# sp-uhh/audio-visual-vad

Hardware: AMD Instinct MI355X
Metric: AV frame-pairs/sec (fwd+bwd) (higher is better)
Workload: dtype f32; 1 GPU; AV_net fused training step (WaveNet-W0 encoder + ResNet-18 trunk + concat + 2xLSTM1024 + FC, masked BCE, backward, RCCL all-reduce, fused Adam): BASELINE configs[3]/[4] per-GPU shard; per_gpu_frame_pairs=1024, global_frame_pairs=1024, sequences_per_gpu=64, parallelism=dp1, reserved_cus=0, reported_block=median

## Files before the change

audio-visual-vad_amd/csrc/wavenet.hip:

```cpp
#include "gemm_api.h"
#include "wn_block.h"
#include "wn_tail.h"

namespace {

static inline int grid1(long n) { long b = (n + 255) / 256; return (int)(b > 8192 ? 8192 : (b < 1 ? 1 : b)); }

__global__ void conv1d_fwd_generic(const float* __restrict__ x, const float* __restrict__ w, const float* __restrict__ bias,
                                   const float* __restrict__ res, float* __restrict__ y, int B, int Cin, int Cout, int Lin,
                                   int Lout, int fw, int dil, int relu_in, int res_off, int res_L) {
  const long n = (long)B * Cout * Lout;
  for (long i = (long)blockIdx.x * blockDim.x + threadIdx.x; i < n; i += (long)gridDim.x * blockDim.x) {
    const int t = (int)(i % Lout);
    const int co = (int)((i / Lout) % Cout);
    const int b = (int)(i / ((long)Lout * Cout));
    float acc = bias ? bias[co] : 0.f;
    const float* xb = x + (long)b * Cin * Lin + t;
    const float* wr = w + (long)co * Cin * fw;
    for (int ci = 0; ci < Cin; ++ci)
      for (int k = 0; k < fw; ++k) {
        float v = xb[(long)ci * Lin + k * dil];
        if (relu_in) v = fmaxf(v, 0.f);
        acc = fmaf(wr[ci * fw + k], v, acc);
      }
// ... 29 lines not shown
  const int c = blockIdx.x;
  float s = 0.f;
  for (int b = blockIdx.y; b < B; b += gridDim.y) {
    const float* p = dy + ((long)b * C + c) * L;
    for (int t = threadIdx.x; t < L; t += 256) s += p[t];
  }
  sm[threadIdx.x] = s;
  __syncthreads();
  for (int o = 128; o > 0; o >>= 1) {
    if (threadIdx.x < o) sm[threadIdx.x] += sm[threadIdx.x + o];
    __syncthreads();
  }
  if (threadIdx.x == 0) db[c] += sm[0];
}

__global__ void __launch_bounds__(256)
    narrow_conv1d_grads(const float* __restrict__ dy, const float* __restrict__ x, float* __restrict__ part,
                        int B, int Cout, int Cin, int Lout, int Lin, int fw) {
  __shared__ float sm[5][256];
  const int co = blockIdx.x, nw = Cin * fw;
  float acc[5] = {0.f, 0.f, 0.f, 0.f, 0.f};
  for (int b = blockIdx.y; b < B; b += gridDim.y) {
    const float* p = dy + ((long)b * Cout + co) * Lout;
    const float* xb = x + (long)b * Cin * Lin;
    for (int t = threadIdx.x; t < Lout; t += 256) {
      const float g = p[t];
      acc[4] += g;
#pragma unroll
      for (int j = 0; j < 4; ++j)
        if (j < nw) acc[j] = fmaf(g, xb[(long)(j / fw) * Lin + t + (j % fw)], acc[j]);
    }
  }
#pragma unroll
  for (int j = 0; j < 5; ++j) sm[j][threadIdx.x] = acc[j];
  __syncthreads();
  for (int o = 128; o > 0; o >>= 1) {
    if (threadIdx.x < o)
#pragma unroll
      for (int j = 0; j < 5; ++j) sm[j][threadIdx.x] += sm[j][threadIdx.x + o];
    __syncthreads();
  }
  if (threadIdx.x < 5) part[((long)blockIdx.y * Cout + co) * 5 + threadIdx.x] = sm[threadIdx.x][0];
}
__global__ void narrow_conv1d_grads_sum(const float* __restrict__ part, int ny, int Cout, int nw, float* __restrict__ dw,
                                        float* __restrict__ db) {
  const int i = blockIdx.x * blockDim.x + threadIdx.x;
  if (i >= Cout * 5) return;
  const int co = i / 5, j = i - co * 5;
  float s = 0.f;
  for (int y = 0; y < ny; ++y) s += part[((long)y * Cout + co) * 5 + j];
  if (j < 4) { if (j < nw && dw) dw[(long)co * nw + j] += s; }
  else if (db) db[co] += s;
}

template <int MODE>
__global__ void __launch_bounds__(256)
    wn_block_fwd_mfma(const float* __restrict__ s_in, const float* __restrict__ w_dil, const float* __restrict__ b_dil,
                      const float* __restrict__ w_dense, const float* __restrict__ b_dense, float* __restrict__ s_out,
                      float* __restrict__ z_out, int B, int Lin, int dil) {
  static_assert(MODE == 0 || MODE == 2, "s_out only, or z only");
  const int lane = threadIdx.x & 63;
  const int li = lane & 31, lh = lane >> 5;
  const int Lo = Lin - dil;
  const int tiles_per_seq = tiles_per_sequence<32>(Lo);
  const long ntiles = (long)B * tiles_per_seq;
// ... 831 lines not shown
  if (threadIdx.x >= 32 || nslab <= 0) return;
  if (i < 2048) { if (tab.dW_dil[l]) tab.dW_dil[l][(i & 1023) * 2 + (i >> 10)] += s; }
  else if (i < 3072) { if (tab.dW_dense[l]) tab.dW_dense[l][i - 2048] += s; }
  else if (i < 3104) { if (tab.db_dil[l]) tab.db_dil[l][i - 3072] += s; }
  else if (tab.db_dense[l]) tab.db_dense[l][i - 3104] += s;
}

struct Plan {
  int n;
  int L[66];
  size_t s[66];
  size_t z, dz, ga, gb, dzt;
  size_t zs[66];
  size_t slab;
  size_t gslab;
  size_t total;
};
static int make_plan(const avvad_wavenet_desc* d, Plan* p) {
  if (!d || d->n_layers < 0 || d->n_layers > 64 || d->B <= 0 || d->fw < 1 || d->qc < 1 || d->R < 1 || d->D < 1 ||
      d->Bn < 1 || d->P < 1 || (d->n_layers > 0 && !d->dilations_h))
    return AVVAD_EINVAL;
  p->n = d->n_layers;
  p->L[0] = d->L - (d->fw - 1);
  for (int i = 0; i < p->n; ++i) p->L[i + 1] = p->L[i] - d->dilations_h[i] * (d->fw - 1);
  if (p->L[p->n] < 1) return AVVAD_EINVAL;
  size_t off = 0;
  auto take = [&](size_t n) { size_t o = off; off += align_up(n, 64); return o; };
  const size_t B = d->B;
  if (d->save_for_backward) {
    for (int i = 0; i <= p->n; ++i) p->s[i] = take(B * d->R * p->L[i]);
    const size_t big = B * (size_t)(d->R > d->D ? d->R : d->D) * p->L[0];
    p->z = take(big); p->dz = take(big); p->ga = take(big); p->gb = take(big);
    p->dzt = take(B * d->Bn * p->L[p->n]);
    {
      const size_t zb = (d->R == 32 && d->D == 32 && d->fw == 2 && p->n > 0) ? take(B * d->D * p->L[1]) : 0;
      for (int i = 0; i < p->n; ++i) p->zs[i] = zb;
    }
    {
      const bool perlayer = d->R == 32 && d->D == 32 && d->fw == 2;
      const size_t a = (size_t)WG_MAXBLK * WG_SLAB * (perlayer ? (size_t)p->n : 1), b2 = (size_t)TAIL_MAXBLK * tail_slab_floats(d->Bn);
      p->slab = take(a > b2 ? a : b2);
    }
    p->gslab = take(igemm::SLAB_FLOATS);
  } else {
    for (int i = 0; i < p->n; ++i) p->zs[i] = 0;
    const size_t a = take(B * d->R * p->L[0]), b2 = take(B * d->R * p->L[0]);
    for (int i = 0; i <= p->n; ++i) p->s[i] = (i & 1) ? b2 : a;
    p->z = take(B * d->D * p->L[0]);
    p->dz = p->ga = p->gb = p->dzt = 0;
  }
  p->total = off;
  return AVVAD_OK;
}

static inline bool mfma_shape(const avvad_wavenet_desc* d) { return d->R == 32 && d->D == 32 && d->fw == 2; }
static inline bool buf_ok(int B, int Lin) {
  return avvad_tune().wn_flat != 1 && (long)Lin * 32 * 4 + 4096 < (1L << 31) && (long)B * cdiv(Lin, 32) < (1L << 31);
}

enum class FwdForm { FLAT, BUF, OCC, WIDE, DMA };
enum class DxForm { FLAT, BUF, OCC };
enum class BwdForm { RESIDENT, OCC, TRANSPOSED, UNFUSED };
enum class TailFwdForm { GENERIC, MFMA1, MFMA4 };
enum class TailBwdForm { PAIR, FUSED, MFMA, GENERIC };
struct FwdChoice { FwdForm form; int grid; };
struct DxChoice { DxForm form; int grid; };
struct BwdChoice { BwdForm form; int grid; int grid_z, grid_dz; };
struct TailFwdChoice { TailFwdForm form; int grid; };
struct TailBwdChoice { TailBwdForm form; int grid; };
// ... 84 lines not shown
  const int ktiles = cdiv(K, igemm::BK);
  int split = 1024 / (cdiv(Cout, 64) * cdiv(Cin * fw, 64));
  if (split > ktiles) split = ktiles;
  if (split < 1) split = 1;
  igemm::RowSegK a{dy, Lout, (long)Cout * Lout, Cout, (int)K, Lout, 0, 0, 1, 0};
  igemm::RowSegK b{x, Lin, (long)Cin * Lin, Cin * fw, (int)K, Lout, 0, relu_in, fw, dil};
  igemm::EpiStore e{dw, (long)Cin * fw, nullptr, 1};
  return igemm::launch<64, 64>(a, b, e, Cout, Cin * fw, (int)K, split, s, slab);
}

static void bias_grad(const float* dy, float* db, int B, int C, int L, hipStream_t s) {
  if (!db) return;
  hipLaunchKernelGGL(chan_sum_acc, dim3(C, 1), dim3(256), 0, s, dy, db, B, C, L);
}

static void launch_tail_fwd(const float* sN, const float* wb, const float* bb, float* out, int B, int R, int Bn, int Lv, int P,
                            hipStream_t s) {
  const TailFwdChoice c = tail_fwd_form(B, R, Bn, P);
  switch (c.form) {
    case TailFwdForm::MFMA4: hipLaunchKernelGGL(tail_fwd_mfma<4>, dim3(c.grid), dim3(256), 0, s, sN, wb, bb, out, B, Bn, Lv, P); break;
    case TailFwdForm::MFMA1: hipLaunchKernelGGL(tail_fwd_mfma<1>, dim3(c.grid), dim3(256), 0, s, sN, wb, bb, out, B, Bn, Lv, P); break;
    case TailFwdForm::GENERIC: hipLaunchKernelGGL(tail_fwd_generic, dim3(P, B), dim3(256), 0, s, sN, wb, bb, out, R, Bn, Lv, P); break;
  }
}

static int launch_tail_bwd(const float* sN, const float* wb, const float* bb, const float* dout, float* dW, float* db, float* dS,
                           float* dzt, float* slab, float* gslab, int B, int R, int Bn, int Lv, int P, hipStream_t s) {
  const TailBwdChoice c = tail_bwd_form(B, Lv, R, Bn, P, dW || db);
  int rc;
  if (c.form == TailBwdForm::PAIR || c.form == TailBwdForm::FUSED) {
    const bool pair = c.form == TailBwdForm::PAIR;
    const size_t lds = (size_t)tail_fused_lds_floats(Bn, pair ? 2 : 1) * sizeof(float);
    if ((rc = pair ? allow_large_lds<tail_bwd_wgrad_pair<8>>(lds, lds) : allow_large_lds<tail_bwd_wgrad_mfma<8>>(lds, lds))) return rc;
    hipLaunchKernelGGL(pair ? tail_bwd_wgrad_pair<8> : tail_bwd_wgrad_mfma<8>, dim3(c.grid), dim3(pair ? 512 : 256), lds, s, sN, wb,
                       bb, dout, dS, slab, B, Lv, P);
    hipLaunchKernelGGL(tail_wgrad_reduce, dim3(cdiv(tail_slab_floats(Bn), 32)), dim3(256), 0, s, slab, c.grid, Bn, dW, db);
    return AVVAD_OK;
  }
  if (c.form == TailBwdForm::MFMA)
    hipLaunchKernelGGL(tail_bwd_mfma, dim3(c.grid), dim3(256), (size_t)tail_wimg_floats(Bn) * sizeof(float), s, sN, wb, bb, dout,
                       dzt, dS, B, Bn, Lv, P);
  else
    hipLaunchKernelGGL(tail_bwd_dz_generic, dim3(grid1((long)B * Bn * Lv)), dim3(256), 0, s, sN, wb, bb, dout, dzt, B, R, Bn, Lv, P);
  if (dW && (rc = wgrad_conv1d(dzt, sN, dW, B, Bn, R, Lv, Lv, 1, 1, 0, s, gslab))) return rc;
  bias_grad(dzt, db, B, Bn, Lv, s);
  if (c.form == TailBwdForm::GENERIC)
    hipLaunchKernelGGL(conv1d_bwd_data_generic, dim3(grid1((long)B * R * Lv)), dim3(256), 0, s, dzt, wb, (const float*)nullptr,
                       (const float*)nullptr, dS, B, R, Bn, Lv, Lv, 1, 1, 0, 0);
  return AVVAD_OK;
}

}

extern "C" size_t avvad_wavenet_workspace(const avvad_wavenet_desc* d) {
  Plan p;
  if (make_plan(d, &p)) return 0;
  return p.total * sizeof(float);
}

extern "C" int avvad_wavenet_fwd(const float* wave, const avvad_wavenet_params* prm, float* out, const avvad_wavenet_desc* d,
                                 void* wsv, size_t ws_bytes, avvad_stream_t sv) {
  AVVAD_ENTER();
  Plan p;
  if (!wave || !prm || !out || !wsv || ws_misaligned(wsv) || make_plan(d, &p)) return AVVAD_EINVAL;
  if (ws_bytes < p.total * sizeof(float)) return AVVAD_EWORKSPACE;
  hipStream_t s = (hipStream_t)sv;
  float* ws = (float*)wsv;
  const int B = d->B, R = d->R, D = d->D, fw = d->fw;
  hipLaunchKernelGGL(conv1d_fwd_generic, dim3(grid1((long)B * R * p.L[0])), dim3(256), 0, s, wave, prm->causal_w,
                     d->use_bias ? prm->causal_b : (const float*)nullptr, (const float*)nullptr, ws + p.s[0], B, d->qc, R,
                     d->L, p.L[0], fw, 1, 0, 0, 0);
  for (int i = 0; i < p.n; ++i) {
    const int dil = d->dilations_h[i];
    const float* bd = d->use_bias ? prm->dil_b_h[i] : nullptr;
    const float* be = d->use_bias ? prm->dense_b_h[i] : nullptr;
    if (mfma_shape(d)) {
      launch_block_fwd(ws + p.s[i], prm->dil_w_h[i], bd, prm->dense_w_h[i], be, ws + p.s[i + 1], B, p.L[i], dil, s);
    } else {
      float* z = ws + p.z;
      hipLaunchKernelGGL(conv1d_fwd_generic, dim3(grid1((long)B * D * p.L[i + 1])), dim3(256), 0, s, ws + p.s[i],
                         prm->dil_w_h[i], bd, (const float*)nullptr, z, B, R, D, p.L[i], p.L[i + 1], fw, dil, 1, 0, 0);
      hipLaunchKernelGGL(conv1d_fwd_generic, dim3(grid1((long)B * R * p.L[i + 1])), dim3(256), 0, s, z, prm->dense_w_h[i], be,
                         ws + p.s[i], ws + p.s[i + 1], B, D, R, p.L[i + 1], p.L[i + 1], 1, 1, 1, p.L[i] - p.L[i + 1], p.L[i]);
    }
  }
  launch_tail_fwd(ws + p.s[p.n], prm->bott_w, d->use_bias ? prm->bott_b : (const float*)nullptr, out, B, R, d->Bn, p.L[p.n],
                  d->P, s);
  AVVAD_LAUNCH_CHECK();
  return AVVAD_OK;
}

extern "C" int avvad_wavenet_block_fwd(const float* s_in, const float* w_dil, const float* b_dil, const float* w_dense,
                                       const float* b_dense, float* s_out, int B, int Lin, int dil, avvad_stream_t sv) {
  AVVAD_ENTER();
  if (!s_in || !w_dil || !w_dense || !s_out || B <= 0 || dil < 1 || Lin - dil < 1) return AVVAD_EINVAL;
  launch_block_fwd(s_in, w_dil, b_dil, w_dense, b_dense, s_out, B, Lin, dil, (hipStream_t)sv);
  AVVAD_LAUNCH_CHECK();
  return AVVAD_OK;
}

extern "C" int avvad_wavenet_bwd(const float* wave, const avvad_wavenet_params* prm, const float* dout,
                                 const avvad_wavenet_grads* g, float* dwave, const avvad_wavenet_desc* d, void* wsv,
                                 size_t ws_bytes, avvad_stream_t sv) {
  AVVAD_ENTER();
  Plan p;
  if (!wave || !prm || !dout || !g || !wsv || ws_misaligned(wsv) || make_plan(d, &p) || !d->save_for_backward) return AVVAD_EINVAL;
  if (ws_bytes < p.total * sizeof(float)) return AVVAD_EWORKSPACE;
  hipStream_t s = (hipStream_t)sv;
  float* ws = (float*)wsv;
  const int B = d->B, R = d->R, D = d->D, fw = d->fw, Bn = d->Bn;
  int rc;
  float* Z = ws + p.z;
  float* DZ = ws + p.dz;
  float* GA = ws + p.ga;
  float* GB = ws + p.gb;
  if ((rc = launch_tail_bwd(ws + p.s[p.n], prm->bott_w, d->use_bias ? prm->bott_b : (const float*)nullptr, dout, g->bott_w,
                            d->use_bias ? g->bott_b : (float*)nullptr, GA, ws + p.dzt, ws + p.slab, ws + p.gslab, B, R, Bn,
                            p.L[p.n], d->P, s)))
    return rc;
  WgradTab wtab;
  bool any_slab = false;
  for (int l = 0; l < WN_MAXL; ++l) {
    wtab.slab[l] = nullptr; wtab.nslab[l] = 0;
    wtab.dW_dil[l] = wtab.db_dil[l] = wtab.dW_dense[l] = wtab.db_dense[l] = nullptr;
  }
  auto note_slabs = [&](int i, float* slab_i, int wb) {
    wtab.slab[i] = slab_i; wtab.nslab[i] = wb;
    wtab.dW_dil[i] = g->dil_w_h[i]; wtab.dW_dense[i] = g->dense_w_h[i];
    wtab.db_dil[i] = d->use_bias ? g->dil_b_h[i] : (float*)nullptr;
    wtab.db_dense[i] = d->use_bias ? g->dense_b_h[i] : (float*)nullptr;
    any_slab = true;
// ... 47 lines not shown
          break;
      }
    } else {
      if (g->dense_w_h[i] && (rc = wgrad_conv1d(GA, Zi, g->dense_w_h[i], B, R, D, Lo, Lo, 1, 1, 1, s, ws + p.gslab))) return rc;
      if (d->use_bias) bias_grad(GA, g->dense_b_h[i], B, R, Lo, s);
      hipLaunchKernelGGL(conv1d_bwd_data_generic, dim3(grid1((long)B * D * Lo)), dim3(256), 0, s, GA, prm->dense_w_h[i], Zi,
                         (const float*)nullptr, DZ, B, D, R, Lo, Lo, 1, 1, 0, 0);
      if (g->dil_w_h[i] && (rc = wgrad_conv1d(DZ, si, g->dil_w_h[i], B, D, R, Lo, Li, fw, dil, 1, s, ws + p.gslab))) return rc;
      if (d->use_bias) bias_grad(DZ, g->dil_b_h[i], B, D, Lo, s);
      hipLaunchKernelGGL(conv1d_bwd_data_generic, dim3(grid1((long)B * R * Li)), dim3(256), 0, s, DZ, prm->dil_w_h[i], si, GA,
                         GB, B, R, D, Li, Lo, fw, dil, Li - Lo, Lo);
    }
    float* t = GA; GA = GB; GB = t;
  }
  if (any_slab) hipLaunchKernelGGL(wn_wgrad_reduce_all, dim3(WG_SLAB / 32, p.n), dim3(256), 0, s, wtab);
  if (d->qc * fw <= 4) {
    if (g->causal_w || (d->use_bias && g->causal_b))
    {
      const int ny = B < 32 ? B : 32;
      float* part = ws + p.gslab;
      hipLaunchKernelGGL(narrow_conv1d_grads, dim3(R, ny), dim3(256), 0, s, GA, wave, part, B, R, d->qc, p.L[0], d->L, fw);
      hipLaunchKernelGGL(narrow_conv1d_grads_sum, dim3(cdiv(R * 5, 256)), dim3(256), 0, s, part, ny, R, d->qc * fw, g->causal_w,
                         d->use_bias ? g->causal_b : (float*)nullptr);
    }
  } else {
    if (g->causal_w && (rc = wgrad_conv1d(GA, wave, g->causal_w, B, R, d->qc, p.L[0], d->L, fw, 1, 0, s, ws + p.gslab))) return rc;
    if (d->use_bias) bias_grad(GA, g->causal_b, B, R, p.L[0], s);
  }
  if (dwave)
    hipLaunchKernelGGL(conv1d_bwd_data_generic, dim3(grid1((long)B * d->qc * d->L)), dim3(256), 0, s, GA, prm->causal_w,
                       (const float*)nullptr, (const float*)nullptr, dwave, B, d->qc, R, d->L, p.L[0], fw, 1, 0, 0);
  AVVAD_LAUNCH_CHECK();
  return AVVAD_OK;
}
```

audio-visual-vad_amd/csrc/wn_tail.h:

```cpp
#pragma once
#include "common.h"

namespace {

constexpr int TAIL_MAXBLK = 256;
constexpr int TAIL_PITCH = 33;
constexpr int TAIL_TILE = 32 * TAIL_PITCH;
constexpr int tail_wimg_floats(int Bn) { return Bn * TAIL_PITCH; }
constexpr int tail_slab_floats(int Bn) { return Bn * 32 + Bn; }
constexpr int tail_fused_lds_floats(int Bn, int WPT) {
  return tail_wimg_floats(Bn) + tail_slab_floats(Bn) + 4 * WPT * 2 * TAIL_TILE + (WPT == 2 ? 4 * TAIL_TILE : 0);
}

__device__ __forceinline__ void pool_bin(int p, int Lv, int P, int& a, int& e) {
  a = (int)(((long)p * Lv) / P);
  e = (int)((((long)(p + 1)) * Lv + P - 1) / P);
}
__device__ __forceinline__ void stage_tail_weights(float* img, const float* __restrict__ wb, int Bn, int tid, int nthreads) {
  for (int i = tid; i < Bn * 32; i += nthreads) img[(i >> 5) * TAIL_PITCH + (i & 31)] = wb[i];
}
struct PoolWindow { int pb[3]; float pc[3]; };
__device__ __forceinline__ PoolWindow pool_window(int t, bool ok, int Lv, int P) {
  PoolWindow w;
  const int c0 = ok ? (int)(((long)t * P) / Lv) : 0;
#pragma unroll
  for (int j = 0; j < 3; ++j) {
    const int p = c0 - 1 + j;
    int a = 0, e = 0;
    const bool in = ok && p >= 0 && p < P;
    if (in) pool_bin(p, Lv, P, a, e);
    const bool hit = in && t >= a && t < e;
    w.pb[j] = hit ? p : 0;
    w.pc[j] = hit ? 1.f / (float)(e - a) : 0.f;
  }
  return w;
}
__device__ __forceinline__ f32x16 tail_z_tile(const float* wl, const float* __restrict__ bb, int nb, const float (&x)[16], int li, int lh) {
  f32x16 accZ;
#pragma unroll
  for (int r = 0; r < 16; ++r) accZ[r] = bb ? bb[nb + mfma32_row(r, lh)] : 0.f;
  float wz[16];
#pragma unroll
  for (int k = 0; k < 16; ++k) wz[k] = wl[(nb + li) * TAIL_PITCH + 2 * k + lh];
#pragma unroll
  for (int k = 0; k < 16; ++k) accZ = mfma32(wz[k], x[k], accZ);
  return accZ;
}
template <class Fetch>
__device__ __forceinline__ void tail_dz_tile(const f32x16& accZ, Fetch fetch, float (&dz)[16]) {
#pragma unroll
  for (int r = 0; r < 16; ++r) { const float g = fetch(r); dz[r] = accZ[r] > 0.f ? g : 0.f; }
}
__device__ __forceinline__ void tail_wt_frag(const float* wl, int nb, int li, int lh, float (&wt)[16]) {
#pragma unroll
  for (int k = 0; k < 16; ++k) wt[k] = wl[(nb + mfma32_row(k, lh)) * TAIL_PITCH + li];
}
__device__ __forceinline__ void tail_ds_product(f32x16& accS, const float (&wt)[16], const float (&dz)[16]) {
#pragma unroll
  for (int r = 0; r < 16; ++r) accS = mfma32(wt[r], dz[r], accS);
}
template <bool DLAYOUT>
__device__ __forceinline__ void tile_to_fragment(float* T, const float (&v)[16], float (&f)[16], int li, int lh) {
  __builtin_amdgcn_wave_barrier();
#pragma unroll
  for (int k = 0; k < 16; ++k) T[(DLAYOUT ? mfma32_row(k, lh) : 2 * k + lh) * TAIL_PITCH + li] = v[k];
  __builtin_amdgcn_wave_barrier();
// ... 53 lines not shown
    const float* sb = s + (long)b * R * Lv + t;
    for (int c = 0; c < R; ++c) z = fmaf(wb[(long)bn * R + c], sb[(long)c * Lv], z);
    float g = 0.f;
    if (z > 0.f) {
      const int p0 = (int)(((long)t * P) / Lv), p1 = (int)((((long)t + 1) * P + Lv - 1) / Lv);
      for (int p = p0; p < p1; ++p) {
        int a, e;
        pool_bin(p, Lv, P, a, e);
        g += dout[((long)b * Bn + bn) * P + p] / (float)(e - a);
      }
    }
    dz[i] = g;
  }
}

template <int NT>
__global__ void __launch_bounds__(256)
    tail_fwd_mfma(const float* __restrict__ s, const float* __restrict__ wb, const float* __restrict__ bb,
                  float* __restrict__ out, int B, int Bn, int Lv, int P) {
  const int lane = threadIdx.x & 63;
  const int li = lane & 31, lh = lane >> 5;
  const int ngrp = Bn / (32 * NT);
  const long nitems = (long)B * P * ngrp;
  const long nwaves = ((long)gridDim.x * blockDim.x) >> 6;
  for (long item = ((long)blockIdx.x * blockDim.x + threadIdx.x) >> 6; item < nitems; item += nwaves) {
    const int grp = (int)(item % ngrp);
    const int p = (int)((item / ngrp) % P);
    const int b = (int)(item / ((long)ngrp * P));
    const int bn0 = grp * 32 * NT;
    int a, e;
    pool_bin(p, Lv, P, a, e);
    float w[NT][16], bias[NT], sum[NT];
#pragma unroll
    for (int n = 0; n < NT; ++n) {
#pragma unroll
      for (int k = 0; k < 16; ++k) w[n][k] = wb[(long)(bn0 + n * 32 + li) * 32 + 2 * k + lh];
      bias[n] = bb ? bb[bn0 + n * 32 + li] : 0.f;
      sum[n] = 0.f;
    }
    const float* sp = s + (long)b * 32 * Lv;
    for (int t0 = a; t0 < e; t0 += 32) {
      const int t = t0 + li;
      const bool ok = t < e;
      const int tcl = ok ? t : a;
      float x[16];
#pragma unroll
      for (int k = 0; k < 16; ++k) x[k] = sp[(long)(2 * k + lh) * Lv + tcl];
#pragma unroll
      for (int k = 0; k < 16; ++k) x[k] = ok ? x[k] : 0.f;
#pragma unroll
      for (int n = 0; n < NT; ++n) {
        f32x16 acc = {};
#pragma unroll
        for (int k = 0; k < 16; ++k) acc = mfma32(x[k], w[n][k], acc);
#pragma unroll
        for (int r = 0; r < 16; ++r)
          if (t0 + mfma32_row(r, lh) < e) sum[n] += relu1(acc[r] + bias[n]);
      }
    }
    const float inv = 1.f / (float)(e - a);
#pragma unroll
    for (int n = 0; n < NT; ++n) {
      const float v = sum[n] + __shfl_xor(sum[n], 32, 64);
      if (lh == 0) out[((long)b * Bn + bn0 + n * 32 + li) * P + p] = v * inv;
    }
  }
}

__global__ void __launch_bounds__(256)
    tail_bwd_mfma(const float* __restrict__ s, const float* __restrict__ wb, const float* __restrict__ bb,
                  const float* __restrict__ dout, float* __restrict__ dzt, float* __restrict__ dS, int B, int Bn, int Lv, int P) {
  const int lane = threadIdx.x & 63;
  const int li = lane & 31, lh = lane >> 5;
  const int tiles_per_seq = (Lv + 31) >> 5;
  const long ntiles = (long)B * tiles_per_seq;
  const long nwaves = ((long)gridDim.x * blockDim.x) >> 6;
  extern __shared__ float wl[];
  stage_tail_weights(wl, wb, Bn, threadIdx.x, 256);
  __syncthreads();
  for (long tile = ((long)blockIdx.x * blockDim.x + threadIdx.x) >> 6; tile < ntiles; tile += nwaves) {
    const int b = (int)(tile / tiles_per_seq);
    const int t = (int)(tile - (long)b * tiles_per_seq) * 32 + li;
    const bool ok = t < Lv;
    const float* sp = s + (long)b * 32 * Lv + (ok ? t : 0);
    float x[16];
#pragma unroll
    for (int k = 0; k < 16; ++k) x[k] = sp[(long)(2 * k + lh) * Lv];
#pragma unroll
    for (int k = 0; k < 16; ++k) x[k] = ok ? x[k] : 0.f;
    const PoolWindow pw = pool_window(t, ok, Lv, P);
    f32x16 accS = {};
    for (int nb = 0; nb < Bn; nb += 32) {
      const f32x16 accZ = tail_z_tile(wl, bb, nb, x, li, lh);
      float dz[16];
      tail_dz_tile(accZ, [&](int r) {
        const long o = ((long)b * Bn + nb + mfma32_row(r, lh)) * P;
        float g = 0.f;
#pragma unroll
        for (int j = 0; j < 3; ++j) g = fmaf(dout[o + pw.pb[j]], pw.pc[j], g);
        return g;
      }, dz);
#pragma unroll
      for (int r = 0; r < 16; ++r)
        if (ok) dzt[((long)b * Bn + nb + mfma32_row(r, lh)) * Lv + t] = dz[r];
      float wt[16];
      tail_wt_frag(wl, nb, li, lh, wt);
      tail_ds_product(accS, wt, dz);
    }
#pragma unroll
    for (int r = 0; r < 16; ++r)
      if (ok) dS[((long)b * 32 + mfma32_row(r, lh)) * Lv + t] = accS[r];
  }
}

template <int NBT, int WPT>
__device__ __forceinline__ void tail_bwd_wgrad_body(const float* __restrict__ s, const float* __restrict__ wb,
                                                    const float* __restrict__ bb, const float* __restrict__ dout,
                                                    float* __restrict__ dS, float* __restrict__ slab, int B, int Lv, int P) {
  static_assert((WPT == 1 || WPT == 2) && NBT % WPT == 0, "one wave per time tile, or two that halve the bottleneck rows");
  constexpr int Bn = NBT * 32, NH = NBT / WPT, NWAVES = 4 * WPT, NTHREADS = 64 * NWAVES, SLAB = tail_slab_floats(Bn);
  extern __shared__ float wl[];
  float* red = wl + tail_wimg_floats(Bn);
  float* tiles = red + SLAB;
  const int lane = threadIdx.x & 63, wave = threadIdx.x >> 6;
  const int li = lane & 31, lh = lane >> 5;
  const int pair = wave >> 1, half = WPT == 2 ? wave & 1 : 0;
  const int tiles_per_seq = (Lv + 31) >> 5;
  const long ntiles = (long)B * tiles_per_seq;
  float *T0 = tiles + wave * 2 * TAIL_TILE, *T1 = T0 + TAIL_TILE;
  float* PS = tiles + (NWAVES * 2 + pair) * TAIL_TILE;
  stage_tail_weights(wl, wb, Bn, threadIdx.x, NTHREADS);
  for (int i = threadIdx.x; i < SLAB; i += NTHREADS) red[i] = 0.f;
// ... 2 lines not shown
  float bsum[NH] = {};
  const int rowV = Lv * 4;
  const bool single = (Lv % P) == 0;
  auto one_tile = [&](long tile, bool live) __attribute__((always_inline)) {
    const int b = __builtin_amdgcn_readfirstlane((int)((live ? tile : 0) / tiles_per_seq));
    const int t = (int)((live ? tile : 0) - (long)b * tiles_per_seq) * 32 + li;
    const bool ok = live && t < Lv;
    const __amdgpu_buffer_rsrc_t rs = brsrc(s + (long)b * 32 * Lv, 32 * rowV);
    const __amdgpu_buffer_rsrc_t rd = brsrc(dS + (long)b * 32 * Lv, 32 * rowV);
    const __amdgpu_buffer_rsrc_t rg = brsrc(dout + (long)b * Bn * P, Bn * P * 4);
    const int offs = ok ? t * 4 + lh * rowV : BUF_OOB;
    const int offd = ok ? t * 4 + 4 * lh * rowV : BUF_OOB;
    float x[16];
#pragma unroll
    for (int k = 0; k < 16; ++k) x[k] = bload(rs, offs, 2 * k * rowV);
    __builtin_amdgcn_sched_barrier(0);
    const PoolWindow pw = pool_window(t, ok, Lv, P);
    int pbo[3];
#pragma unroll
    for (int j = 0; j < 3; ++j) pbo[j] = (pw.pb[j] + 4 * lh * P) * 4;
    float fs[16];
    tile_to_fragment<false>(T0, x, fs, li, lh);
    f32x16 accS = {};
#pragma unroll
    for (int n = 0; n < NH; ++n) {
      const int nb = (half * NH + n) * 32;
      float wt[16];
      if constexpr (WPT == 1) tail_wt_frag(wl, nb, li, lh, wt);
      const f32x16 accZ = tail_z_tile(wl, bb, nb, x, li, lh);
      if constexpr (WPT == 2) __builtin_amdgcn_sched_barrier(0);
      float dz[16];
      tail_dz_tile(accZ, [&](int r) {
        const int row = (nb + mfma32_row(r, 0)) * P * 4;
        if (single) return bload(rg, pbo[1], row) * pw.pc[1];
        float g = 0.f;
#pragma unroll
        for (int j = 0; j < 3; ++j) g = fmaf(bload(rg, pbo[j], row), pw.pc[j], g);
        return g;
      }, dz);
      if constexpr (WPT == 2) {
        __builtin_amdgcn_sched_barrier(0);
        tail_wt_frag(wl, nb, li, lh, wt);
      }
      tail_ds_product(accS, wt, dz);
      if constexpr (WPT == 2) __builtin_amdgcn_sched_barrier(0);
      float fz[16];
      tile_to_fragment<true>(T1, dz, fz, li, lh);
#pragma unroll
      for (int q = 0; q < 16; ++q) bsum[n] += fz[q];
#pragma unroll
      for (int q = 0; q < 16; ++q) accW[n] = mfma32(fz[q], fs[q], accW[n]);
    }
    if constexpr (WPT == 2) {
      if (half == 1) {
#pragma unroll
        for (int r = 0; r < 16; ++r) PS[mfma32_row(r, lh) * TAIL_PITCH + li] = accS[r];
      }
      __syncthreads();
// ... 27 lines not shown
#pragma unroll
    for (int h = 0; h < 2; ++h) {
      if (h == 1) __builtin_amdgcn_wave_barrier();
#pragma unroll
      for (int n = 0; n < NH; ++n)
        if (lh == h) red[Bn * 32 + (half * NH + n) * 32 + li] += bsum[n];
    }
  });
  __syncthreads();
  float* out = slab + (long)blockIdx.x * SLAB;
  for (int i = threadIdx.x; i < SLAB; i += NTHREADS) out[i] = red[i];
}

template <int NBT>
__global__ void __launch_bounds__(256)
    tail_bwd_wgrad_mfma(const float* __restrict__ s, const float* __restrict__ wb, const float* __restrict__ bb,
                        const float* __restrict__ dout, float* __restrict__ dS, float* __restrict__ slab, int B, int Lv, int P) {
  tail_bwd_wgrad_body<NBT, 1>(s, wb, bb, dout, dS, slab, B, Lv, P);
}

template <int NBT>
__global__ void __launch_bounds__(512, 2)
    tail_bwd_wgrad_pair(const float* __restrict__ s, const float* __restrict__ wb, const float* __restrict__ bb,
                        const float* __restrict__ dout, float* __restrict__ dS, float* __restrict__ slab, int B, int Lv, int P) {
  tail_bwd_wgrad_body<NBT, 2>(s, wb, bb, dout, dS, slab, B, Lv, P);
}

__global__ void __launch_bounds__(256)
    tail_wgrad_reduce(const float* __restrict__ slab, int nslab, int Bn, float* __restrict__ dW, float* __restrict__ db) {
  const int n = tail_slab_floats(Bn);
  const int i = blockIdx.x * 32 + (threadIdx.x & 31);
  const float sum = slab_sum_fixed_order(slab + i, i < n ? nslab : 0, n);
  if (threadIdx.x >= 32 || i >= n) return;
  if (i < Bn * 32) { if (dW) dW[i] += sum; }
  else if (db) db[i - Bn * 32] += sum;
}

}
```

Baseline: 60600 frame-pairs/s.

## Save ReLU mask in tail forward; vectorize narrow causal conv fwd and grads

```diff
diff --git a/audio-visual-vad_amd/csrc/wavenet.hip b/audio-visual-vad_amd/csrc/wavenet.hip
--- a/audio-visual-vad_amd/csrc/wavenet.hip
+++ b/audio-visual-vad_amd/csrc/wavenet.hip
@@ -67,41 +67,132 @@
   if (threadIdx.x == 0) db[c] += sm[0];
 }
 
+static inline int narrow_quads(int Lout) { return (Lout + 6) / 4; }
+typedef float f4u __attribute__((ext_vector_type(4), aligned(4)));
+__device__ __forceinline__ void narrow_window(const float* __restrict__ xb, int Cin, int fw, int Lin, int t0, bool whole,
+                                              float (&win)[4][7]) {
+#pragma unroll
+  for (int ci = 0; ci < 4; ++ci) {
+    if (ci >= Cin) continue;
+    const float* xr = xb + ci * Lin;
+    if (whole) {
+      const f4u v = *(const f4u*)(xr + t0);
+      win[ci][0] = v[0]; win[ci][1] = v[1]; win[ci][2] = v[2]; win[ci][3] = v[3];
+#pragma unroll
+      for (int m = 4; m < 7; ++m)
+        if (m < 3 + fw) win[ci][m] = xr[t0 + m];
+    } else {
+#pragma unroll
+      for (int m = 0; m < 7; ++m)
+        if (m < 3 + fw) win[ci][m] = xr[min(max(t0 + m, 0), Lin - 1)];
+    }
+  }
+}
 __global__ void __launch_bounds__(256)
     narrow_conv1d_grads(const float* __restrict__ dy, const float* __restrict__ x, float* __restrict__ part,
-                        int B, int Cout, int Cin, int Lout, int Lin, int fw) {
-  __shared__ float sm[5][256];
-  const int co = blockIdx.x, nw = Cin * fw;
-  float acc[5] = {0.f, 0.f, 0.f, 0.f, 0.f};
-  for (int b = blockIdx.y; b < B; b += gridDim.y) {
-    const float* p = dy + ((long)b * Cout + co) * Lout;
+                        int B, int Cout, int Cin, int Lout, int Lin, int fw, int nbg, int qpc) {
+  __shared__ float sm[5][4];
+  const int co = blockIdx.x;
+  const int bg = blockIdx.y % nbg, chunk = blockIdx.y / nbg;
+  float acc[4][4] = {}, accb = 0.f;
+  for (int b = bg; b < B; b += nbg) {
+    const long row0 = ((long)b * Cout + co) * Lout;
+    const int head = (int)(row0 & 3);
+    const float* p = dy + row0;
     const float* xb = x + (long)b * Cin * Lin;
-    for (int t = threadIdx.x; t < Lout; t += 256) {
-      const float g = p[t];
-      acc[4] += g;
-#pragma unroll
-      for (int j = 0; j < 4; ++j)
-        if (j < nw) acc[j] = fmaf(g, xb[(long)(j / fw) * Lin + t + (j % fw)], acc[j]);
-    }
-  }
-#pragma unroll
-  for (int j = 0; j < 5; ++j) sm[j][threadIdx.x] = acc[j];
+    const int qend = min((chunk + 1) * qpc, (head + Lout + 3) >> 2);
+    for (int q = chunk * qpc + threadIdx.x; q < qend; q += 256) {
+      const int t0 = 4 * q - head;
+      const bool whole = t0 >= 0 && t0 + 4 <= Lout;
+      float g[4], win[4][7];
+      if (whole) {
+        const f4v v = *(const f4v*)(p + t0);
+        g[0] = v[0]; g[1] = v[1]; g[2] = v[2]; g[3] = v[3];
+      } else {
+#pragma unroll
+        for (int i = 0; i < 4; ++i) g[i] = (t0 + i >= 0 && t0 + i < Lout) ? p[t0 + i] : 0.f;
+      }
+      narrow_window(xb, Cin, fw, Lin, t0, whole, win);
+#pragma unroll
+      for (int i = 0; i < 4; ++i) {
+        accb += g[i];
+#pragma unroll
+        for (int ci = 0; ci < 4; ++ci)
+#pragma unroll
+          for (int k = 0; k < 4; ++k)
+            if (ci < Cin && k < fw) acc[ci][k] = fmaf(g[i], win[ci][i + k], acc[ci][k]);
+      }
+    }
+  }
+  auto meet = [&](float v, int j) {
+#pragma unroll
+    for (int o = 32; o > 0; o >>= 1) v += __shfl_xor(v, o, 64);
+    if ((threadIdx.x & 63) == 0) sm[j][threadIdx.x >> 6] = v;
+  };
+#pragma unroll
+  for (int ci = 0; ci < 4; ++ci)
+#pragma unroll
+    for (int k = 0; k < 4; ++k)
+      if (ci < Cin && k < fw) meet(acc[ci][k], ci * fw + k);
+  meet(accb, 4);
   __syncthreads();
-  for (int o = 128; o > 0; o >>= 1) {
-    if (threadIdx.x < o)
-#pragma unroll
-      for (int j = 0; j < 5; ++j) sm[j][threadIdx.x] += sm[j][threadIdx.x + o];
-    __syncthreads();
-  }
-  if (threadIdx.x < 5) part[((long)blockIdx.y * Cout + co) * 5 + threadIdx.x] = sm[threadIdx.x][0];
-}
-__global__ void narrow_conv1d_grads_sum(const float* __restrict__ part, int ny, int Cout, int nw, float* __restrict__ dw,
-                                        float* __restrict__ db) {
-  const int i = blockIdx.x * blockDim.x + threadIdx.x;
-  if (i >= Cout * 5) return;
+  if (threadIdx.x < 5) {
+    const bool used = threadIdx.x == 4 || (int)threadIdx.x < Cin * fw;
+    part[((long)blockIdx.y * Cout + co) * 5 + threadIdx.x] =
+        used ? ((sm[threadIdx.x][0] + sm[threadIdx.x][1]) + sm[threadIdx.x][2]) + sm[threadIdx.x][3] : 0.f;
+  }
+}
+constexpr int NARROW_CO = 4;
+__global__ void __launch_bounds__(256)
+    narrow_conv1d_fwd(const float* __restrict__ x, const float* __restrict__ w, const float* __restrict__ bias,
+                      float* __restrict__ y, int B, int Cin, int Cout, int Lin, int Lout, int fw) {
+  const int q = blockIdx.x * 256 + threadIdx.x;
+  for (int co = blockIdx.y * NARROW_CO; co < min((int)(blockIdx.y + 1) * NARROW_CO, Cout); ++co) {
+    float wr[4][4];
+#pragma unroll
+    for (int ci = 0; ci < 4; ++ci)
+#pragma unroll
+      for (int k = 0; k < 4; ++k) wr[ci][k] = (ci < Cin && k < fw) ? w[(co * Cin + ci) * fw + k] : 0.f;
+    const float b0 = bias ? bias[co] : 0.f;
+    for (int b = blockIdx.z; b < B; b += gridDim.z) {
+      const long row0 = ((long)b * Cout + co) * Lout;
+      const int head = (int)(row0 & 3);
+      const int t0 = 4 * q - head;
+      if (t0 >= Lout) continue;
+      const bool whole = t0 >= 0 && t0 + 4 <= Lout;
+      float win[4][7], v[4];
+      narrow_window(x + (long)b * Cin * Lin, Cin, fw, Lin, t0, whole, win);
+#pragma unroll
+      for (int i = 0; i < 4; ++i) {
+        float acc = b0;
+#pragma unroll
+        for (int ci = 0; ci < 4; ++ci)
+#pragma unroll
+          for (int k = 0; k < 4; ++k)
+            if (ci < Cin && k < fw) acc = fmaf(wr[ci][k], win[ci][i + k], acc);
+        v[i] = acc;
+      }
+      float* p = y + row0;
+      if (whole) {
+        *(f4v*)(p + t0) = f4v{v[0], v[1], v[2], v[3]};
+      } else {
+#pragma unroll
+        for (int i = 0; i < 4; ++i)
+          if (t0 + i >= 0 && t0 + i < Lout) p[t0 + i] = v[i];
+      }
+    }
+  }
+}
+__global__ void __launch_bounds__(64)
+    narrow_conv1d_grads_sum(const float* __restrict__ part, int ny, int Cout, int nw, float* __restrict__ dw,
+                            float* __restrict__ db) {
+  const int i = blockIdx.x;
   const int co = i / 5, j = i - co * 5;
   float s = 0.f;
-  for (int y = 0; y < ny; ++y) s += part[((long)y * Cout + co) * 5 + j];
+  for (int y = threadIdx.x; y < ny; y += 64) s += part[((long)y * Cout + co) * 5 + j];
+#pragma unroll
+  for (int o = 32; o > 0; o >>= 1) s += __shfl_xor(s, o, 64);
+  if (threadIdx.x != 0) return;
   if (j < 4) { if (j < nw && dw) dw[(long)co * nw + j] += s; }
   else if (db) db[co] += s;
 }
@@ -963,8 +1054,11 @@
   size_t zs[66];
   size_t slab;
   size_t gslab;
+  size_t tmask;
+  bool has_tmask;
   size_t total;
 };
+static inline bool tail_has_mask(const avvad_wavenet_desc* d) { return d->save_for_backward && d->R == 32 && d->Bn % 32 == 0; }
 static int make_plan(const avvad_wavenet_desc* d, Plan* p) {
   if (!d || d->n_layers < 0 || d->n_layers > 64 || d->B <= 0 || d->fw < 1 || d->qc < 1 || d->R < 1 || d->D < 1 ||
       d->Bn < 1 || d->P < 1 || (d->n_layers > 0 && !d->dilations_h))
@@ -991,17 +1085,22 @@
       p->slab = take(a > b2 ? a : b2);
     }
     p->gslab = take(igemm::SLAB_FLOATS);
+    p->has_tmask = tail_has_mask(d);
+    p->tmask = p->has_tmask ? take(tail_mask_words(B, d->Bn, p->L[p->n])) : 0;
   } else {
     for (int i = 0; i < p->n; ++i) p->zs[i] = 0;
     const size_t a = take(B * d->R * p->L[0]), b2 = take(B * d->R * p->L[0]);
     for (int i = 0; i <= p->n; ++i) p->s[i] = (i & 1) ? b2 : a;
     p->z = take(B * d->D * p->L[0]);
     p->dz = p->ga = p->gb = p->dzt = 0;
+    p->has_tmask = false;
+    p->tmask = 0;
   }
   p->total = off;
   return AVVAD_OK;
 }
 
+static inline bool narrow_causal(const avvad_wavenet_desc* d) { return d->qc * d->fw <= 4 && d->R <= 2048; }
 static inline bool mfma_shape(const avvad_wavenet_desc* d) { return d->R == 32 && d->D == 32 && d->fw == 2; }
 static inline bool buf_ok(int B, int Lin) {
   return avvad_tune().wn_flat != 1 && (long)Lin * 32 * 4 + 4096 < (1L << 31) && (long)B * cdiv(Lin, 32) < (1L << 31);
@@ -1116,31 +1215,38 @@
   hipLaunchKernelGGL(chan_sum_acc, dim3(C, 1), dim3(256), 0, s, dy, db, B, C, L);
 }
 
-static void launch_tail_fwd(const float* sN, const float* wb, const float* bb, float* out, int B, int R, int Bn, int Lv, int P,
-                            hipStream_t s) {
+static int launch_tail_fwd(const float* sN, const float* wb, const float* bb, float* out, unsigned* mask, int B, int R, int Bn,
+                           int Lv, int P, hipStream_t s) {
   const TailFwdChoice c = tail_fwd_form(B, R, Bn, P);
-  switch (c.form) {
-    case TailFwdForm::MFMA4: hipLaunchKernelGGL(tail_fwd_mfma<4>, dim3(c.grid), dim3(256), 0, s, sN, wb, bb, out, B, Bn, Lv, P); break;
-    case TailFwdForm::MFMA1: hipLaunchKernelGGL(tail_fwd_mfma<1>, dim3(c.grid), dim3(256), 0, s, sN, wb, bb, out, B, Bn, Lv, P); break;
-    case TailFwdForm::GENERIC: hipLaunchKernelGGL(tail_fwd_generic, dim3(P, B), dim3(256), 0, s, sN, wb, bb, out, R, Bn, Lv, P); break;
-  }
-}
-
-static int launch_tail_bwd(const float* sN, const float* wb, const float* bb, const float* dout, float* dW, float* db, float* dS,
-                           float* dzt, float* slab, float* gslab, int B, int R, int Bn, int Lv, int P, hipStream_t s) {
+  if (c.form == TailFwdForm::GENERIC) {
+    hipLaunchKernelGGL(tail_fwd_generic, dim3(P, B), dim3(256), 0, s, sN, wb, bb, out, R, Bn, Lv, P);
+    return AVVAD_OK;
+  }
+  const int mask_or = mask && !tail_mask_aligned(Lv, P);
+  if (mask_or && hipMemsetAsync(mask, 0, tail_mask_words(B, Bn, Lv) * sizeof(unsigned), s) != hipSuccess) return AVVAD_ELAUNCH;
+  const size_t lds = Bn <= TAIL_FWD_STAGE_BN ? (size_t)tail_wimg_floats(Bn) * sizeof(float) : 0;
+  hipLaunchKernelGGL(c.form == TailFwdForm::MFMA4 ? tail_fwd_mfma<4> : tail_fwd_mfma<1>, dim3(c.grid), dim3(256), lds, s, sN, wb, bb,
+                     out, mask, mask_or, B, Bn, Lv, P);
+  return AVVAD_OK;
+}
+
+static int launch_tail_bwd(const float* sN, const float* wb, const float* bb, const unsigned* mask, const float* dout, float* dW,
+                           float* db, float* dS, float* dzt, float* slab, float* gslab, int B, int R, int Bn, int Lv, int P,
+                           hipStream_t s) {
   const TailBwdChoice c = tail_bwd_form(B, Lv, R, Bn, P, dW || db);
   int rc;
+  if (c.form != TailBwdForm::GENERIC && !mask) return AVVAD_EINVAL;
   if (c.form == TailBwdForm::PAIR || c.form == TailBwdForm::FUSED) {
     const bool pair = c.form == TailBwdForm::PAIR;
     const size_t lds = (size_t)tail_fused_lds_floats(Bn, pair ? 2 : 1) * sizeof(float);
     if ((rc = pair ? allow_large_lds<tail_bwd_wgrad_pair<8>>(lds, lds) : allow_large_lds<tail_bwd_wgrad_mfma<8>>(lds, lds))) return rc;
     hipLaunchKernelGGL(pair ? tail_bwd_wgrad_pair<8> : tail_bwd_wgrad_mfma<8>, dim3(c.grid), dim3(pair ? 512 : 256), lds, s, sN, wb,
-                       bb, dout, dS, slab, B, Lv, P);
+                       mask, dout, dS, slab, B, Lv, P);
     hipLaunchKernelGGL(tail_wgrad_reduce, dim3(cdiv(tail_slab_floats(Bn), 32)), dim3(256), 0, s, slab, c.grid, Bn, dW, db);
     return AVVAD_OK;
   }
   if (c.form == TailBwdForm::MFMA)
-    hipLaunchKernelGGL(tail_bwd_mfma, dim3(c.grid), dim3(256), (size_t)tail_wimg_floats(Bn) * sizeof(float), s, sN, wb, bb, dout,
+    hipLaunchKernelGGL(tail_bwd_mfma, dim3(c.grid), dim3(256), (size_t)tail_wimg_floats(Bn) * sizeof(float), s, mask, wb, dout,
                        dzt, dS, B, Bn, Lv, P);
   else
     hipLaunchKernelGGL(tail_bwd_dz_generic, dim3(grid1((long)B * Bn * Lv)), dim3(256), 0, s, sN, wb, bb, dout, dzt, B, R, Bn, Lv, P);
@@ -1169,9 +1275,14 @@
   hipStream_t s = (hipStream_t)sv;
   float* ws = (float*)wsv;
   const int B = d->B, R = d->R, D = d->D, fw = d->fw;
-  hipLaunchKernelGGL(conv1d_fwd_generic, dim3(grid1((long)B * R * p.L[0])), dim3(256), 0, s, wave, prm->causal_w,
-                     d->use_bias ? prm->causal_b : (const float*)nullptr, (const float*)nullptr, ws + p.s[0], B, d->qc, R,
-                     d->L, p.L[0], fw, 1, 0, 0, 0);
+  if (narrow_causal(d))
+    hipLaunchKernelGGL(narrow_conv1d_fwd, dim3(cdiv(narrow_quads(p.L[0]), 256), cdiv(R, NARROW_CO), B < 65535 ? B : 65535), dim3(256), 0, s, wave,
+                       prm->causal_w, d->use_bias ? prm->causal_b : (const float*)nullptr, ws + p.s[0], B, d->qc, R, d->L,
+                       p.L[0], fw);
+  else
+    hipLaunchKernelGGL(conv1d_fwd_generic, dim3(grid1((long)B * R * p.L[0])), dim3(256), 0, s, wave, prm->causal_w,
+                       d->use_bias ? prm->causal_b : (const float*)nullptr, (const float*)nullptr, ws + p.s[0], B, d->qc, R,
+                       d->L, p.L[0], fw, 1, 0, 0, 0);
   for (int i = 0; i < p.n; ++i) {
     const int dil = d->dilations_h[i];
     const float* bd = d->use_bias ? prm->dil_b_h[i] : nullptr;
@@ -1186,8 +1297,10 @@
                          ws + p.s[i], ws + p.s[i + 1], B, D, R, p.L[i + 1], p.L[i + 1], 1, 1, 1, p.L[i] - p.L[i + 1], p.L[i]);
     }
   }
-  launch_tail_fwd(ws + p.s[p.n], prm->bott_w, d->use_bias ? prm->bott_b : (const float*)nullptr, out, B, R, d->Bn, p.L[p.n],
-                  d->P, s);
+  int rc;
+  if ((rc = launch_tail_fwd(ws + p.s[p.n], prm->bott_w, d->use_bias ? prm->bott_b : (const float*)nullptr, out,
+                            p.has_tmask ? (unsigned*)(ws + p.tmask) : nullptr, B, R, d->Bn, p.L[p.n], d->P, s)))
+    return rc;
   AVVAD_LAUNCH_CHECK();
   return AVVAD_OK;
 }
@@ -1216,7 +1329,8 @@
   float* DZ = ws + p.dz;
   float* GA = ws + p.ga;
   float* GB = ws + p.gb;
-  if ((rc = launch_tail_bwd(ws + p.s[p.n], prm->bott_w, d->use_bias ? prm->bott_b : (const float*)nullptr, dout, g->bott_w,
+  if ((rc = launch_tail_bwd(ws + p.s[p.n], prm->bott_w, d->use_bias ? prm->bott_b : (const float*)nullptr,
+                            p.has_tmask ? (const unsigned*)(ws + p.tmask) : nullptr, dout, g->bott_w,
                             d->use_bias ? g->bott_b : (float*)nullptr, GA, ws + p.dzt, ws + p.slab, ws + p.gslab, B, R, Bn,
                             p.L[p.n], d->P, s)))
     return rc;
@@ -1294,13 +1408,14 @@
     float* t = GA; GA = GB; GB = t;
   }
   if (any_slab) hipLaunchKernelGGL(wn_wgrad_reduce_all, dim3(WG_SLAB / 32, p.n), dim3(256), 0, s, wtab);
-  if (d->qc * fw <= 4) {
+  if (narrow_causal(d)) {
     if (g->causal_w || (d->use_bias && g->causal_b))
     {
-      const int ny = B < 32 ? B : 32;
+      const int nbg = B < 32 ? B : 32, nq = narrow_quads(p.L[0]);
+      const int nchunk = nq / 512 < 1 ? 1 : (nq / 512 > 16 ? 16 : nq / 512), qpc = cdiv(nq, nchunk), ny = nbg * nchunk;
       float* part = ws + p.gslab;
-      hipLaunchKernelGGL(narrow_conv1d_grads, dim3(R, ny), dim3(256), 0, s, GA, wave, part, B, R, d->qc, p.L[0], d->L, fw);
-      hipLaunchKernelGGL(narrow_conv1d_grads_sum, dim3(cdiv(R * 5, 256)), dim3(256), 0, s, part, ny, R, d->qc * fw, g->causal_w,
+      hipLaunchKernelGGL(narrow_conv1d_grads, dim3(R, ny), dim3(256), 0, s, GA, wave, part, B, R, d->qc, p.L[0], d->L, fw, nbg, qpc);
+      hipLaunchKernelGGL(narrow_conv1d_grads_sum, dim3(R * 5), dim3(64), 0, s, part, ny, R, d->qc * fw, g->causal_w,
                          d->use_bias ? g->causal_b : (float*)nullptr);
     }
   } else {
diff --git a/audio-visual-vad_amd/csrc/wn_tail.h b/audio-visual-vad_amd/csrc/wn_tail.h
--- a/audio-visual-vad_amd/csrc/wn_tail.h
+++ b/audio-visual-vad_amd/csrc/wn_tail.h
@@ -35,21 +35,22 @@
   }
   return w;
 }
-__device__ __forceinline__ f32x16 tail_z_tile(const float* wl, const float* __restrict__ bb, int nb, const float (&x)[16], int li, int lh) {
-  f32x16 accZ;
-#pragma unroll
-  for (int r = 0; r < 16; ++r) accZ[r] = bb ? bb[nb + mfma32_row(r, lh)] : 0.f;
-  float wz[16];
-#pragma unroll
-  for (int k = 0; k < 16; ++k) wz[k] = wl[(nb + li) * TAIL_PITCH + 2 * k + lh];
-#pragma unroll
-  for (int k = 0; k < 16; ++k) accZ = mfma32(wz[k], x[k], accZ);
-  return accZ;
-}
+inline size_t tail_mask_words(size_t B, int Bn, int Lv) { return B * (size_t)((Lv + 31) >> 5) * (size_t)Bn; }
+inline bool tail_mask_aligned(int Lv, int P) { return Lv % P == 0 && (Lv / P) % 32 == 0; }
+__device__ __forceinline__ bool tail_z_positive(float z) { return __builtin_bit_cast(int, z) > 0; }
 template <class Fetch>
-__device__ __forceinline__ void tail_dz_tile(const f32x16& accZ, Fetch fetch, float (&dz)[16]) {
-#pragma unroll
-  for (int r = 0; r < 16; ++r) { const float g = fetch(r); dz[r] = accZ[r] > 0.f ? g : 0.f; }
+__device__ __forceinline__ void tail_dz_tile(unsigned mw, Fetch fetch, float (&dz)[16], int li, int lh) {
+#pragma unroll
+  for (int r = 0; r < 16; ++r) {
+    const float g = fetch(r);
+    const unsigned w0 = __builtin_amdgcn_readlane(mw, mfma32_row(r, 0)), w1 = __builtin_amdgcn_readlane(mw, mfma32_row(r, 1));
+    dz[r] = (((lh ? w1 : w0) >> li) & 1u) ? g : 0.f;
+  }
+}
+__device__ __forceinline__ float tail_row_value(float v, int r, int lh) {
+  const int v0 = __builtin_amdgcn_readlane(__builtin_bit_cast(int, v), mfma32_row(r, 0));
+  const int v1 = __builtin_amdgcn_readlane(__builtin_bit_cast(int, v), mfma32_row(r, 1));
+  return __builtin_bit_cast(float, lh ? v1 : v0);
 }
 __device__ __forceinline__ void tail_wt_frag(const float* wl, int nb, int li, int lh, float (&wt)[16]) {
 #pragma unroll
@@ -133,15 +134,23 @@
   }
 }
 
+constexpr int TAIL_FWD_STAGE_BN = 256;
 template <int NT>
 __global__ void __launch_bounds__(256)
     tail_fwd_mfma(const float* __restrict__ s, const float* __restrict__ wb, const float* __restrict__ bb,
-                  float* __restrict__ out, int B, int Bn, int Lv, int P) {
+                  float* __restrict__ out, unsigned* __restrict__ mask, int mask_or, int B, int Bn, int Lv, int P) {
   const int lane = threadIdx.x & 63;
   const int li = lane & 31, lh = lane >> 5;
   const int ngrp = Bn / (32 * NT);
   const long nitems = (long)B * P * ngrp;
   const long nwaves = ((long)gridDim.x * blockDim.x) >> 6;
+  const int tiles_per_seq = (Lv + 31) >> 5;
+  extern __shared__ float wl[];
+  const bool staged = Bn <= TAIL_FWD_STAGE_BN;
+  if (staged) {
+    stage_tail_weights(wl, wb, Bn, threadIdx.x, 256);
+    __syncthreads();
+  }
   for (long item = ((long)blockIdx.x * blockDim.x + threadIdx.x) >> 6; item < nitems; item += nwaves) {
     const int grp = (int)(item % ngrp);
     const int p = (int)((item / ngrp) % P);
@@ -152,8 +161,13 @@
     float w[NT][16], bias[NT], sum[NT];
 #pragma unroll
     for (int n = 0; n < NT; ++n) {
-#pragma unroll
-      for (int k = 0; k < 16; ++k) w[n][k] = wb[(long)(bn0 + n * 32 + li) * 32 + 2 * k + lh];
+      if (staged) {
+#pragma unroll
+        for (int k = 0; k < 16; ++k) w[n][k] = wl[(bn0 + n * 32 + li) * TAIL_PITCH + 2 * k + lh];
+      } else {
+#pragma unroll
+        for (int k = 0; k < 16; ++k) w[n][k] = wb[(long)(bn0 + n * 32 + li) * 32 + 2 * k + lh];
+      }
       bias[n] = bb ? bb[bn0 + n * 32 + li] : 0.f;
       sum[n] = 0.f;
     }
@@ -172,9 +186,28 @@
         f32x16 acc = {};
 #pragma unroll
         for (int k = 0; k < 16; ++k) acc = mfma32(x[k], w[n][k], acc);
+        unsigned bits = 0;
 #pragma unroll
         for (int r = 0; r < 16; ++r)
-          if (t0 + mfma32_row(r, lh) < e) sum[n] += relu1(acc[r] + bias[n]);
+          if (t0 + mfma32_row(r, lh) < e) {
+            const float z = acc[r] + bias[n];
+            sum[n] += relu1(z);
+            bits |= tail_z_positive(z) ? 1u << mfma32_row(r, lh) : 0u;
+          }
+        if (mask) {
+          bits |= (unsigned)__shfl_xor((int)bits, 32, 64);
+          unsigned* mw = mask + ((long)b * tiles_per_seq + (t0 >> 5)) * Bn + bn0 + n * 32 + li;
+          if (lh == 0) {
+            if (!mask_or) {
+              *mw = bits;
+            } else {
+              const int sh = t0 & 31;
+              const unsigned lo = bits << sh, hi = sh ? bits >> (32 - sh) : 0u;
+              if (lo) atomicOr(mw, lo);
+              if (hi) atomicOr(mw + Bn, hi);
+            }
+          }
+        }
       }
     }
     const float inv = 1.f / (float)(e - a);
@@ -187,8 +220,8 @@
 }
 
 __global__ void __launch_bounds__(256)
-    tail_bwd_mfma(const float* __restrict__ s, const float* __restrict__ wb, const float* __restrict__ bb,
-                  const float* __restrict__ dout, float* __restrict__ dzt, float* __restrict__ dS, int B, int Bn, int Lv, int P) {
+    tail_bwd_mfma(const unsigned* __restrict__ mask, const float* __restrict__ wb, const float* __restrict__ dout,
+                  float* __restrict__ dzt, float* __restrict__ dS, int B, int Bn, int Lv, int P) {
   const int lane = threadIdx.x & 63;
   const int li = lane & 31, lh = lane >> 5;
   const int tiles_per_seq = (Lv + 31) >> 5;
@@ -201,24 +234,17 @@
     const int b = (int)(tile / tiles_per_seq);
     const int t = (int)(tile - (long)b * tiles_per_seq) * 32 + li;
     const bool ok = t < Lv;
-    const float* sp = s + (long)b * 32 * Lv + (ok ? t : 0);
-    float x[16];
-#pragma unroll
-    for (int k = 0; k < 16; ++k) x[k] = sp[(long)(2 * k + lh) * Lv];
-#pragma unroll
-    for (int k = 0; k < 16; ++k) x[k] = ok ? x[k] : 0.f;
     const PoolWindow pw = pool_window(t, ok, Lv, P);
     f32x16 accS = {};
     for (int nb = 0; nb < Bn; nb += 32) {
-      const f32x16 accZ = tail_z_tile(wl, bb, nb, x, li, lh);
       float dz[16];
-      tail_dz_tile(accZ, [&](int r) {
+      tail_dz_tile(mask[tile * Bn + nb + li], [&](int r) {
         const long o = ((long)b * Bn + nb + mfma32_row(r, lh)) * P;
         float g = 0.f;
 #pragma unroll
         for (int j = 0; j < 3; ++j) g = fmaf(dout[o + pw.pb[j]], pw.pc[j], g);
         return g;
-      }, dz);
+      }, dz, li, lh);
 #pragma unroll
       for (int r = 0; r < 16; ++r)
         if (ok) dzt[((long)b * Bn + nb + mfma32_row(r, lh)) * Lv + t] = dz[r];
@@ -234,7 +260,7 @@
 
 template <int NBT, int WPT>
 __device__ __forceinline__ void tail_bwd_wgrad_body(const float* __restrict__ s, const float* __restrict__ wb,
-                                                    const float* __restrict__ bb, const float* __restrict__ dout,
+                                                    const unsigned* __restrict__ mask, const float* __restrict__ dout,
                                                     float* __restrict__ dS, float* __restrict__ slab, int B, int Lv, int P) {
   static_assert((WPT == 1 || WPT == 2) && NBT % WPT == 0, "one wave per time tile, or two that halve the bottleneck rows");
   constexpr int Bn = NBT * 32, NH = NBT / WPT, NWAVES = 4 * WPT, NTHREADS = 64 * NWAVES, SLAB = tail_slab_floats(Bn);
@@ -267,11 +293,20 @@
     float x[16];
 #pragma unroll
     for (int k = 0; k < 16; ++k) x[k] = bload(rs, offs, 2 * k * rowV);
+    unsigned mw[NH];
+#pragma unroll
+    for (int n = 0; n < NH; ++n) mw[n] = mask[(live ? tile : 0) * Bn + (half * NH + n) * 32 + li];
     __builtin_amdgcn_sched_barrier(0);
     const PoolWindow pw = pool_window(t, ok, Lv, P);
     int pbo[3];
 #pragma unroll
     for (int j = 0; j < 3; ++j) pbo[j] = (pw.pb[j] + 4 * lh * P) * 4;
+    const int p0 = __builtin_amdgcn_readfirstlane(pw.pb[1]);
+    const bool whole =
+        __builtin_amdgcn_ballot_w64(ok && pw.pc[0] == 0.f && pw.pc[2] == 0.f && pw.pc[1] != 0.f && pw.pb[1] == p0) == ~0ull;
+    float gv[NH];
+#pragma unroll
+    for (int n = 0; n < NH; ++n) gv[n] = bload(rg, whole ? (((half * NH + n) * 32 + li) * P + p0) * 4 : BUF_OOB, 0) * pw.pc[1];
     float fs[16];
     tile_to_fragment<false>(T0, x, fs, li, lh);
     f32x16 accS = {};
@@ -279,22 +314,18 @@
     for (int n = 0; n < NH; ++n) {
       const int nb = (half * NH + n) * 32;
       float wt[16];
-      if constexpr (WPT == 1) tail_wt_frag(wl, nb, li, lh, wt);
-      const f32x16 accZ = tail_z_tile(wl, bb, nb, x, li, lh);
-      if constexpr (WPT == 2) __builtin_amdgcn_sched_barrier(0);
       float dz[16];
-      tail_dz_tile(accZ, [&](int r) {
+      if (whole) tail_dz_tile(mw[n], [&](int r) { return tail_row_value(gv[n], r, lh); }, dz, li, lh);
+      else tail_dz_tile(mw[n], [&](int r) {
         const int row = (nb + mfma32_row(r, 0)) * P * 4;
         if (single) return bload(rg, pbo[1], row) * pw.pc[1];
         float g = 0.f;
 #pragma unroll
         for (int j = 0; j < 3; ++j) g = fmaf(bload(rg, pbo[j], row), pw.pc[j], g);
         return g;
-      }, dz);
-      if constexpr (WPT == 2) {
-        __builtin_amdgcn_sched_barrier(0);
-        tail_wt_frag(wl, nb, li, lh, wt);
-      }
+      }, dz, li, lh);
+      if constexpr (WPT == 2) __builtin_amdgcn_sched_barrier(0);
+      tail_wt_frag(wl, nb, li, lh, wt);
       tail_ds_product(accS, wt, dz);
       if constexpr (WPT == 2) __builtin_amdgcn_sched_barrier(0);
       float fz[16];
@@ -352,16 +383,16 @@
 
 template <int NBT>
 __global__ void __launch_bounds__(256)
-    tail_bwd_wgrad_mfma(const float* __restrict__ s, const float* __restrict__ wb, const float* __restrict__ bb,
+    tail_bwd_wgrad_mfma(const float* __restrict__ s, const float* __restrict__ wb, const unsigned* __restrict__ mask,
                         const float* __restrict__ dout, float* __restrict__ dS, float* __restrict__ slab, int B, int Lv, int P) {
-  tail_bwd_wgrad_body<NBT, 1>(s, wb, bb, dout, dS, slab, B, Lv, P);
+  tail_bwd_wgrad_body<NBT, 1>(s, wb, mask, dout, dS, slab, B, Lv, P);
 }
 
 template <int NBT>
 __global__ void __launch_bounds__(512, 2)
-    tail_bwd_wgrad_pair(const float* __restrict__ s, const float* __restrict__ wb, const float* __restrict__ bb,
+    tail_bwd_wgrad_pair(const float* __restrict__ s, const float* __restrict__ wb, const unsigned* __restrict__ mask,
                         const float* __restrict__ dout, float* __restrict__ dS, float* __restrict__ slab, int B, int Lv, int P) {
-  tail_bwd_wgrad_body<NBT, 2>(s, wb, bb, dout, dS, slab, B, Lv, P);
+  tail_bwd_wgrad_body<NBT, 2>(s, wb, mask, dout, dS, slab, B, Lv, P);
 }
 
 __global__ void __launch_bounds__(256)
```

After: 60960 frame-pairs/s, median of 6. About the same (+0.6%).
